# omnirevolve/omnirevolve-image-processor

Hardware: AMD Instinct MI355X
Metric: Mpx/s end-to-end (color->order) (higher is better)
Workload: dtype u8/i32 raster + f32/f64 geometry; 1 GPU; 4096x4096 BGR image, 8 colour layers, stages 02->12 (k-means fit, masks, edges, contours, scale, sort, intra dedup, cross dedup, plot order), default A4 canvas 8400x11880; parallelism=one GPU, one pipeline per colour layer, ops_last_step_rank0=4261, exchange=none

## Files before the change

### omnirevolve-image-processor_amd/csrc/orip_ctx.h

```cpp
#pragma once

#include <hip/hip_runtime.h>
#include <cstdint>
#include <cstdio>
#include <cstring>
#include <string>
#include <vector>
#include <map>
#include <mutex>
#include <atomic>
#include "../../include/orip.h"

typedef uint8_t u8;

#define ORIP_FAIL_AS(ctx, who, ...)                                      \
    do {                                                                 \
        char _b[512];                                                    \
        snprintf(_b, sizeof(_b), __VA_ARGS__);                           \
        { std::lock_guard<std::mutex> _g((ctx)->mu); (ctx)->err = std::string(who) + ": " + _b; } \
        return -1;                                                       \
    } while (0)
#define ORIP_FAIL(ctx, ...) ORIP_FAIL_AS(ctx, __func__, __VA_ARGS__)

#define HIPC_AS(ctx, who, call)                                                                \
// ... 72 lines not shown
    struct { void* pp; size_t off; } slot[CAP]; int n = 0; size_t total = 0;
    template <class T> void take(T*& ptr, size_t count, size_t align = 16) {
        if (alignof(T) > align) align = alignof(T);
        total = (total + align - 1) / align * align;
        if (n < CAP) { slot[n].pp = &ptr; slot[n].off = total; }
        n++; total += count * sizeof(T);
    }
    template <class... T> void each(size_t count, T*&... ptrs) { (take(ptrs, count), ...); }
    hipError_t commit(DBuf& buf, size_t tail_bytes) {
        const hipError_t e = n > CAP ? hipErrorInvalidValue : buf.ensure(total + tail_bytes);
        for (int i = 0; e == hipSuccess && i < n; i++) { void* a = (char*)buf.p + slot[i].off; memcpy(slot[i].pp, &a, sizeof a); }
        return e;
    }
};

struct LaneFlags {
    int not_binary;
    uint8_t palette[ORIP_MAX_LAYERS * 3];
    alignas(8) unsigned long long palette_counts[ORIP_MAX_LAYERS];
    alignas(8) unsigned long long label_counts[ORIP_MAX_LAYERS];
    int thin_changed[2];
    unsigned chain_counts[2];
    int trace_overflow;
    int nn_seed[2];
    alignas(8) unsigned long long nn_dbg2[10];
    int caps_overflow;
    unsigned caps_distinct;
    unsigned accept_survivors;
    alignas(8) unsigned long long accept_work;
    int zs_changed[12];
    unsigned comp_counts[3];
    int taps_kept;
    int plot_ops;
};
static_assert(sizeof(LaneFlags) <= 4096, "LaneRes::flags is 4096 bytes, allocated and zeroed by orip_create");

enum { VT0_KEYS = 0, VT0_HEADS = 1, VT0_COMP_START = 2, VT0_ORDER = 3, VT0_ORDER_SORT = 5, VT0_MEMO = 6, VT0_LOG_USED = 7, VT0_WINFO = 8, VT0_EDGE_BITS = 10,
       VT0_NMS_BITS = 11 };
enum { VTL_RANKS = 0,
       VTL_CUM = 1,
       VTL_SPLIT = 2,
       VTL_SAMPLES = 3,
       VTL_CAPS = 4,
       VTL_CELLS = 5,
       VTL_FEAT = 6,
       VTL_RUN_STARTS = 7,
       VTL_TAIL_RUNS = 8,
       VTL_STEPLOG = 9,
       VTL_SPLIT_FEAT = 10,
       VT_LEAVES = 11,
       VT_SLOTS = 12 };
struct LaneRes {
    hipStream_t stream = 0;
    hipStream_t stream2 = 0;
    hipEvent_t ev2 = nullptr, ev3 = nullptr, ev4 = nullptr;
    DBuf vtmp[VT_SLOTS], tmpE, tmpF, flags, canvas;
    DBuf pixbits;
    unsigned caps_hint = 0;
    hipEvent_t ev0 = nullptr, ev1 = nullptr;
    DPolys tp[6];
    struct Prefetch08 {
        bool pending = false;
        bool valid = false; uint64_t tag = 0; int64_t n = 0; int64_t tot_f = 0; double step = 0;
        const int64_t* src_off = nullptr;
        DBuf seg;
        DBuf feat, info, cum, ord;
// ... 130 lines not shown
```

### omnirevolve-image-processor_amd/csrc/vector08a.hip

```cpp
#include "vec08.h"
#include <rocprim/rocprim.hpp>
#include <type_traits>
#include <vector>

namespace {

template <class Src>
__global__ __launch_bounds__(128) void k_split_small08(Src src, int64_t n_polys, orip_params08 P, const PolyFeat* __restrict__ feat,
                                                        unsigned* __restrict__ is_tap, unsigned* __restrict__ is_keep, int2* __restrict__ tap_xy, GatherDesc* __restrict__ kd) {
    int64_t i = (int64_t)blockIdx.x * blockDim.x + threadIdx.x;
    if (i > n_polys) return;
    if (i == n_polys) { is_tap[i] = 0; is_keep[i] = 0; return; }
    const int64_t n = src.len(i);
    unsigned tap = 0, keep = 0;
    GatherDesc g; g.begin = src.off[i]; g.len = n; g.rev = 0; g.src = (int32_t)i;
    if (n >= 2) {
        const int32_t x0 = feat[i].x0, x1 = feat[i].x1, y0 = feat[i].y0, y1 = feat[i].y1;
        double d = (double)max(x1 - x0, y1 - y0);
        if (d <= P.tap_diam && d <= P.tap_max_dim && n <= (int64_t)P.tap_max_v) {
            double per; float cx, cy, r;
            if constexpr (std::is_same<Src, ESrc>::value) {
                const int32_t* p = reinterpret_cast<const int32_t*>(src.pts + src.off[i]);
                per = (double)vs::pairwise_seglen_sum<0>(p, n);
                if (per <= P.tap_max_per) vs::min_enclosing_circle(p, n, cx, cy, r);
            } else {
                auto cu = src.cur(i);
                LocalPts<decltype(cu), 64> lp; lp.load(cu, (int)n);
                per = (double)vs::pairwise_seglen_sum<0>(lp.xy, n);
                if (per <= P.tap_max_per) vs::min_enclosing_circle(lp.xy, n, cx, cy, r);
            }
            if (per <= P.tap_max_per) { tap = 1; tap_xy[i] = make_int2((int)vs::round_half_even((double)cx), (int)vs::round_half_even((double)cy)); }
        }
        if (!tap && !(d < P.min_keep)) {
// ... 368 lines not shown
    __syncthreads();
    const unsigned l0 = threadIdx.x * S;
    double v[S]; unsigned f[S];
#pragma unroll
    for (int q = 0; q < S; q++) { v[q] = shx[smp_slot8(l0 + q)]; f[q] = (b0 + l0 + q < MS) ? shr[smp_slot4(l0 + q)] >> 31 : 0u; }
    double wa = v[0]; unsigned wf = f[0];
#pragma unroll
    for (int q = 1; q < S; q++) { wa = f[q] ? v[q] : __dadd_rn(wa, v[q]); wf |= f[q]; }
    wave_seg_step<0x111, 0xf>(wa, wf); wave_seg_step<0x112, 0xf>(wa, wf); wave_seg_step<0x114, 0xf>(wa, wf); wave_seg_step<0x118, 0xf>(wa, wf);
    wave_seg_step<0x142, 0xa>(wa, wf); wave_seg_step<0x143, 0xc>(wa, wf);
    const int lane = threadIdx.x & 63, wv = threadIdx.x >> 6;
    if (lane == 63) { swa[wv] = wa; swf[wv] = wf; }
    double ea = __hiloint2double(__builtin_amdgcn_update_dpp(0, __double2hiint(wa), 0x138 , 0xf, 0xf, false),
                                 __builtin_amdgcn_update_dpp(0, __double2loint(wa), 0x138, 0xf, 0xf, false));
    const unsigned ef = (unsigned)__builtin_amdgcn_update_dpp(0, (int)wf, 0x138, 0xf, 0xf, false);
    __syncthreads();
    if (!ef) {
        double ca = 0.0;
        for (int k = 0; k < wv; k++) ca = swf[k] ? swa[k] : __dadd_rn(ca, swa[k]);
        ea = __dadd_rn(ca, ea);
    }
#pragma unroll
    for (int q = 0; q < S; q++) { ea = f[q] ? v[q] : __dadd_rn(ea, v[q]); v[q] = ea; }
    const unsigned gs = b0 + l0;
    if (gs + S <= MS) { double2* o = reinterpret_cast<double2*>(A.Sloc + gs); o[0] = make_double2(v[0], v[1]); o[1] = make_double2(v[2], v[3]); }
    else { for (int q = 0; q < S; q++) if (gs + q < MS) A.Sloc[gs + q] = v[q]; }
}

__device__ __forceinline__ double dpp_shr1_f64(double v) {
    const int lo = __builtin_amdgcn_update_dpp(0, __double2loint(v), 0x138 , 0xf, 0xf, true);
    const int hi = __builtin_amdgcn_update_dpp(0, __double2hiint(v), 0x138, 0xf, 0xf, true);
    return __hiloint2double(hi, lo);
}
__global__ __launch_bounds__(64) void k_tail_replay(const unsigned* __restrict__ sbase, int64_t n_rank, double T, SampleArrs A, unsigned* __restrict__ npop, const unsigned* __restrict__ only) {
    constexpr unsigned C = 1024u, RM = 2u * C - 1u;
    __shared__ double ops[64], rr[64];
    __shared__ double Dl[2 * C];
    __shared__ unsigned NPl[C];
    const int lane = threadIdx.x;
    for (int64_t r = blockIdx.x; r < n_rank; r += gridDim.x) {
        if (only && !only[r]) continue;
        const unsigned b = sbase[r], e = sbase[r + 1];
        if (e <= b) continue;
        const double* D = A.dprev + b; unsigned* NP = npop + b;
        const unsigned m = e - b;
        unsigned head = 0; double racc = 0.0;
        unsigned j0 = 0, cb = 0;
        auto fill = [&](unsigned c0) {
            double td[16]; unsigned tn[16];
#pragma unroll
            for (int u = 0; u < 16; u++) { const unsigned idx = c0 + (unsigned)lane + 64u * u; td[u] = D[idx < m ? idx : m - 1u]; tn[u] = NP[idx < m ? idx : m - 1u]; }
#pragma unroll
            for (int u = 0; u < 16; u++) { const unsigned idx = c0 + (unsigned)lane + 64u * u; Dl[idx & RM] = td[u]; NPl[idx & (C - 1u)] = tn[u]; }
        };
        auto dist = [&](unsigned idx) -> double { return (idx + C >= cb && idx < cb + C) ? Dl[idx & RM] : D[idx]; };
        auto plain = [&](unsigned s) {
            if (s > head) racc = __dadd_rn(racc, dist(s));
            while (head <= s && racc > T) { head++; if (head <= s) racc = __dsub_rn(racc, dist(head)); else racc = 0.0; }
            if (lane == 0) NP[s] = head;
        };
        fill(0);
        __syncthreads();
        while (j0 < m) {
            if (j0 >= cb + C) { __syncthreads(); cb += C; fill(cb); __syncthreads(); }
            const unsigned s = j0 + (unsigned)lane; const bool valid = s < m && s < cb + C;
            unsigned hp = valid ? NPl[s & (C - 1u)] : 0u;
            hp = hp > head ? hp : head;
            hp = wave_incl_scan_max_u32(hp);
            unsigned prevh = (unsigned)__builtin_amdgcn_update_dpp(0, (int)hp, 0x138 , 0xf, 0xf, true); if (lane == 0) prevh = head;
            const unsigned np = hp - prevh;
            const unsigned inc = valid ? 1u + np : 0u;
            unsigned off = wave_incl_scan_u32(inc);
            const unsigned long long fitm = __ballot(valid && off <= 64u);
            const int m_fit = __popcll(fitm);
            if (m_fit == 0) { plain(j0); j0++; continue; }
            const unsigned total = (unsigned)__builtin_amdgcn_readlane((int)off, m_fit - 1);
            off -= inc;
            if (lane < m_fit) {
                ops[off] = s > prevh ? dist(s) : 0.0;
                for (unsigned t = 0; t < np; t++) ops[off + 1u + t] = -dist(prevh + 1u + t);
            }
            __syncthreads();
            const double v = (unsigned)lane < total ? ops[lane] : 0.0;
            double d = lane == 0 ? __dadd_rn(racc, v) : v;
            double pre = d;
#pragma unroll
            for (int q = 1; q < 64; q++) pre = __dadd_rn(dpp_shr1_f64(pre), d);
            rr[lane] = pre;
            __syncthreads();
            bool bad = false;
            if (lane < m_fit) {
                const double after = rr[off + np];
                bad = after > T || (np > 0u && !(rr[off + np - 1u] > T)) || hp > s;
            }
            const unsigned long long badm = __ballot(bad);
            const int ncommit = badm ? __ffsll((long long)badm) - 1 : m_fit;
            if (lane < ncommit) NP[s] = hp;
            if (ncommit > 0) {
                head = (unsigned)__builtin_amdgcn_readlane((int)hp, ncommit - 1);
                const unsigned last_op = (unsigned)__builtin_amdgcn_readlane((int)(off + np), ncommit - 1);
                racc = rr[last_op];
            }
            __syncthreads();
            j0 += (unsigned)ncommit;
            if (badm) { plain(j0); j0++; }
        }
        __syncthreads();
    }
}

#define ORIP_TAIL_EPS 1e-6
#define ORIP_TAIL_BLOCKS 32u
__global__ __launch_bounds__(256) void k_tail_par(const unsigned* __restrict__ sbase, const unsigned* __restrict__ rank, const double* __restrict__ Sloc, unsigned MS, double T,
                                                   unsigned* __restrict__ npop, unsigned* __restrict__ redo) {
    __shared__ double win[512];
    const unsigned g0 = blockIdx.x * 256, w0 = g0 >= 256 ? g0 - 256 : 0;
    const unsigned KB = g0 / ORIP_SMP_BLOCK, B0 = KB * ORIP_SMP_BLOCK;
    const double lastprev = w0 < B0 ? Sloc[B0 - 1] : 0.0;
    for (unsigned t = threadIdx.x; t < 512; t += 256) {
        const unsigned idx = w0 + t;
        win[t] = (idx < MS && idx < g0 + 256) ? (idx < B0 ? Sloc[idx] - lastprev : Sloc[idx]) : 0.0;
    }
    __syncthreads();
    unsigned g = g0 + threadIdx.x;
    if (g >= MS) return;
    const unsigned r = rank[g], b = sbase[r];
    const double Sj = Sloc[g];
    bool unsure = !(Sj + (b < B0 ? lastprev : 0.0) < 4194304.0) || (g - b) >= (1u << 20);
    unsigned kc = KB; double acc = 0.0;
    auto tail = [&](unsigned p) -> double {
        if (p >= w0) return Sj - win[p - w0];
        const unsigned kb = p / ORIP_SMP_BLOCK;
        if (KB - kb > ORIP_TAIL_BLOCKS) { unsure = true; return __longlong_as_double(0x7ff0000000000000LL); }
        if (kb > kc) { kc = KB; acc = 0.0; }
        while (kc > kb) { kc--; acc += Sloc[kc * ORIP_SMP_BLOCK + (ORIP_SMP_BLOCK - 1u)]; }
        const double up = Sj + acc;
        if (!(up < 4194304.0)) unsure = true;
        return up - Sloc[p];
    };
    unsigned lo = b, hi = g;
    const unsigned wlo = max(b, w0);
    if (wlo == b || !(tail(wlo) <= T)) {
        if (wlo > b) lo = wlo + 1;
        else if (tail(b) <= T) hi = b;
        while (lo < hi) { const unsigned mid = (lo + hi) >> 1; if (tail(mid) <= T) hi = mid; else lo = mid + 1; }
    } else {
        hi = wlo;
        for (unsigned stepb = 1; hi > b; stepb <<= 1) {
            const unsigned p = (hi - b > stepb) ? hi - stepb : b;
            if (tail(p) <= T) { hi = p; if (p == b) break; } else { lo = p + 1; break; }
        }
        while (lo < hi) { const unsigned mid = (lo + hi) >> 1; if (tail(mid) <= T) hi = mid; else lo = mid + 1; }
    }
    const unsigned h = lo;
    if (!(tail(h) <= T - ORIP_TAIL_EPS)) unsure = true;
    if (h > b && !(tail(h - 1) > T + ORIP_TAIL_EPS)) unsure = true;
    npop[g] = h - b;
    if (unsure) redo[r] = 1u;
}
struct IncIndex {
    const unsigned* pxy;
    __device__ unsigned operator()(unsigned g) const { return pxy[g] != ORIP_PXY_OUT ? g + 1u : 0u; }
};
__global__ __launch_bounds__(256) void k_capprev(const unsigned* __restrict__ sbase, unsigned MS, SampleArrs A, const unsigned* __restrict__ lastin, int* __restrict__ capprev) {
    unsigned g = blockIdx.x * 256 + threadIdx.x;
    if (g >= MS) return;
    if (A.pxy[g] == ORIP_PXY_OUT) { capprev[g] = -2; return; }
    const unsigned b = sbase[A.rank[g]];
    const unsigned l = g > b ? lastin[g - 1] : 0u;
    capprev[g] = l ? (int)(l - 1u - b) : -1;
}

__device__ __forceinline__ unsigned long long cap_key(int x0, int y0, int x1, int y1) {
    unsigned long long a = ((unsigned long long)(unsigned)x0 << 14) | (unsigned)y0, b = ((unsigned long long)(unsigned)x1 << 14) | (unsigned)y1;
    if (b < a) { unsigned long long t = a; a = b; b = t; }
    return ((a << 28) | b) + 1ULL;
}
__device__ __forceinline__ unsigned long long hash64(unsigned long long x) { x ^= x >> 33; x *= 0xff51afd7ed558ccdULL; x ^= x >> 33; x *= 0xc4ceb9fe1a85ec53ULL; x ^= x >> 33; return x; }
struct __attribute__((aligned(16))) CapSlot { unsigned long long key; unsigned val; unsigned pad; };
__global__ __launch_bounds__(256) void k_caps_init(CapSlot* __restrict__ tab, unsigned long long tsize, LaneFlags* __restrict__ fl) {
    unsigned long long i = (unsigned long long)blockIdx.x * 256 + threadIdx.x;
    if (i == 0) { fl->caps_overflow = 0; fl->caps_distinct = 0u; fl->accept_survivors = 0u; fl->accept_work = 0ull; }
    if (i < tsize) reinterpret_cast<uint4*>(tab)[i] = make_uint4(0u, 0u, 0xffffffffu, 0u);
}
constexpr int ORIP_CAPSSET_PROBES = 4;
constexpr int ORIP_CAPSSET_SHIFT = 52;
template <bool CP>
__global__ __launch_bounds__(256) void k_caps_insert(SampleArrs A, const unsigned* __restrict__ sbase, const int* __restrict__ capprev, unsigned MS,
                                                      unsigned chunks, unsigned smask,
                                                      CapSlot* tab, unsigned long long tmask, int max_probe, int* __restrict__ overflow) {
    constexpr int S = 4;
// ... 364 lines not shown
        hipLaunchKernelGGL(k_pf_pick_info, dim3(cdiv(nk, 256)), dim3(256), 0, LN(c).stream, kept0.vview.as<VView>(), nk, F.info.as<RsInfo>(), F.n, F.src_off, F.src_off, F.tot_f, a.info, a.cumoff);
    } else {
        HIPC(c, hipMemcpyAsync(a.cumoff, kept0.off.p, (size_t)(nk + 1) * 8, hipMemcpyDeviceToDevice, LN(c).stream));
        { ProfScope ps(c, "k_cumlen"); ORIP_WITH_SRC(c, kept0, sv, { hipLaunchKernelGGL(k_cumlen<decltype(sv)>, dim3(cdiv(nk, 128)), dim3(128), 0, LN(c).stream, sv, nk, a.step, a.cum, a.info); }); }
        if (kept0.total > ORIP_LONG_CUM) { ProfScope ps(c, "k_cumlen_long"); ORIP_WITH_SRC(c, kept0, sv, {
                hipLaunchKernelGGL(k_cumlen_long2<decltype(sv)>, dim3((unsigned)std::min<int64_t>(nk, 8192), 1), dim3(64), 0, LN(c).stream, sv, nk, a.step, a.cum, (int64_t)0, a.info, a.ord, 0, (const float*)nullptr); }); }
    }
    T.tick("cumlen");
    hipLaunchKernelGGL(k_rank_counts, dim3(cdiv(nk + 1, 256)), dim3(256), 0, LN(c).stream, a.info, a.ord, nk, a.mr, a.feat, W, H, a.sbase + nk + 1, a.redo);
    ORIP_TRY(vscan_excl<unsigned>(c, a.mr, a.sbase, (size_t)nk + 1));
    unsigned ms_out[2] = {0, 0};
    ORIP_TRY(vread(c, ms_out, a.sbase + nk, 2));
    const unsigned MS = a.MS = ms_out[0]; a.any_out = ms_out[1] != 0 || getenv("ORIP_CAPPREV_SCAN");
    if (MS == 0) return 0;
    if (MS > 0x7ffffff0u) ORIP_FAIL(c, "too many samples");
    if (T.on) { char b[48]; snprintf(b, sizeof b, " [MS %u]", MS); T.log += b; }
    { Carve L; L.each(MS, a.A.sx, a.A.sy, a.A.dprev, a.A.pxy, a.A.rank, a.npop, a.capprev, a.sflag); HIPC(c, L.commit(LN(c).vtmp[VTL_SAMPLES], 1024)); }
    { Carve L; L.take(a.A.Sloc, MS); HIPC(c, L.commit(LN(c).vtmp[VTL_TAIL_RUNS], 64)); }
    const unsigned nb = (unsigned)cdiv(MS, 256);
    { Carve L; L.each(MS, a.ckin, a.ckout, a.cvin, a.cvout); L.take(a.hints, nb + 1, 64);
      HIPC(c, L.commit(LN(c).vtmp[VTL_CELLS], 64 + (size_t)MS * 8)); }
    a.cell = P.grid_stride > 0 ? P.grid_stride : std::max(4.0, P.col_rad); a.inv = 1.0 / a.cell;
    a.Wq = (W + 63) >> 6;
    HIPC(c, LN(c).canvas.ensure((size_t)W * H * 4 + 64));
    a.firstseq = LN(c).canvas.as<unsigned>();
    HIPC(c, LN(c).pixbits.ensure((size_t)a.Wq * H * 8 + 64));
    a.pixbits = LN(c).pixbits.as<unsigned long long>();
    HIPC(c, hipMemsetAsync(a.pixbits, 0, (size_t)a.Wq * H * 8, LN(c).stream));
    hipLaunchKernelGGL(k_sample_hints, dim3(cdiv(nb, 256)), dim3(256), 0, LN(c).stream, a.cumoff, a.cum, a.info, a.ord, a.sbase, nk, MS, a.step, nb, a.hints);
    { ProfScope ps(c, "k_samples"); ORIP_WITH_SRC(c, kept0, sv, { hipLaunchKernelGGL(k_samples<decltype(sv)>, dim3(cdiv(nb, 4)), dim3(256), 0, LN(c).stream, sv, a.cumoff, a.cum, a.info, a.ord, a.sbase, nk, MS, a.step, W, H, a.A, a.hints, (unsigned)nb, a.pixbits, a.Wq, a.firstseq); }); }
    T.tick("samples");
    return 0;
}
static void tail_dbg_dump(orip_ctx* c, int layer, const A08& a) {
    const int64_t nk = a.nk;
    std::vector<unsigned> h(nk), sb(nk + 1);
    hipStreamSynchronize(LN(c).stream);
    hipMemcpy(h.data(), a.redo, nk * 4, hipMemcpyDeviceToHost);
    hipMemcpy(sb.data(), a.sbase, (nk + 1) * 4, hipMemcpyDeviceToHost);
    unsigned long long nf = 0, sf = 0, mx = 0;
    for (int64_t q = 0; q < nk; q++) if (h[q]) { nf++; sf += sb[q + 1] - sb[q]; mx = std::max<unsigned long long>(mx, sb[q + 1] - sb[q]); }
    fprintf(stderr, "[tail dbg] layer %d: %llu of %lld polylines redone, %llu of %u samples, longest redone %llu\n", layer, nf, (long long)nk, sf, a.MS, mx);
}
static int a3_tails(orip_ctx* c, int layer, const orip_params08& P, A08& a) {
    const int64_t nk = a.nk; const unsigned MS = a.MS;
    {
        ProfScope ps(c, "k_tail_sim");
        hipLaunchKernelGGL(k_tail_par, dim3(cdiv(MS, 256)), dim3(256), 0, LN(c).stream, a.sbase, a.A.rank, a.A.Sloc, MS, P.tail_len_px, a.npop, a.redo);
        if (getenv("ORIP_TAIL_DBG")) tail_dbg_dump(c, layer, a);
        const unsigned* only = getenv("ORIP_TAIL_SEQ") ? nullptr : a.redo;
        HIPC(c, hipEventRecord(LN(c).ev2, LN(c).stream));
        HIPC(c, hipStreamWaitEvent(LN(c).stream2, LN(c).ev2, 0));
        hipLaunchKernelGGL(k_tail_replay, dim3((unsigned)std::min<int64_t>(nk, 65535)), dim3(64), 0, LN(c).stream2, a.sbase, nk, P.tail_len_px, a.A, a.npop, only);
        HIPC(c, hipEventRecord(LN(c).ev3, LN(c).stream2));
    }
    if (a.any_out) {
        unsigned* lastin = LN(c).vtmp[VTL_TAIL_RUNS].as<unsigned>();
        auto vin = rocprim::make_transform_iterator(rocprim::counting_iterator<unsigned>(0u), IncIndex{a.A.pxy});
        HIPC(c, orip_with_tmp(c, [&](void* tmp, size_t& bytes) { return rocprim::inclusive_scan_by_key(tmp, bytes, a.A.rank, vin, lastin, (size_t)MS, rocprim::maximum<unsigned>(), rocprim::equal_to<unsigned>(), LN(c).stream); }));
        hipLaunchKernelGGL(k_capprev, dim3(cdiv(MS, 256)), dim3(256), 0, LN(c).stream, a.sbase, MS, a.A, lastin, a.capprev);
    }
    else a.capprev = nullptr;
    return 0;
}
static int a4_capsules(orip_ctx* c, const orip_params08& P, A08& a) {
    const unsigned MS = a.MS; LaneFlags* fl = LN(c).flags.as<LaneFlags>();
    unsigned long long tfull = 1024; while (tfull < 2ull * MS) tfull <<= 1;
    unsigned long long tsize = 1024;
    if (LN(c).caps_hint) { while (tsize < 3ull * LN(c).caps_hint) tsize <<= 1; } else { while (tsize < MS / 4ull) tsize <<= 1; }
    tsize = std::min(tsize, tfull);
    if (getenv("ORIP_CAPS_TINY")) tsize = 1024;
    static const unsigned cand[] = {8192u, 4096u, 2048u, 1024u};
    unsigned R = 1024u, TS = 2048u;
    for (unsigned r : cand) if (cdiv(MS, r) >= 2048 || r == 1024u) { R = r; break; }
    if (const char* e = getenv("ORIP_CAPS_RANGE")) {
        char* end = nullptr; const unsigned long r = strtoul(e, &end, 10); unsigned long t = TS;
        if (end && *end == ':') t = strtoul(end + 1, nullptr, 10);
        if (r < 1024 || r > 65536 || (r & 1023)) ORIP_FAIL(c, "ORIP_CAPS_RANGE: a multiple of 1024 up to 65536");
        if (t < 32 || t > 4096 || (t & (t - 1))) ORIP_FAIL(c, "ORIP_CAPS_RANGE: a power of two from 32 to 4096 slots");
        R = (unsigned)r; TS = (unsigned)t;
    }
    if (getenv("ORIP_CAPSSET_TINY")) TS = 32u;
    const unsigned lds = TS * 12u;
    CapSlot* tab = nullptr;
    int* d_ovf = &fl->caps_overflow; unsigned* d_dist = &fl->caps_distinct;
    for (;; tsize = std::min(tfull, tsize * 4)) {
        HIPC(c, LN(c).vtmp[VTL_CAPS].ensure((size_t)tsize * 16 + 64));
// ... 67 lines not shown
```

### omnirevolve-image-processor_amd/csrc/vector08b.hip

```cpp
#include "vec08.h"
#include "bitplane.h"
#include <cstdio>
#define PAD8 64

namespace {

__global__ __launch_bounds__(256) void k_iota(int* a, int n) { int i = blockIdx.x * 256 + threadIdx.x; if (i < n) a[i] = i; }
__global__ __launch_bounds__(256) void k_bbox_pairs(const PolyFeat* __restrict__ f, int n, int exp, int* __restrict__ par) {
    for (int i = blockIdx.x; i < n; i += gridDim.x) {
        int ax0 = f[i].x0 - exp, ay0 = f[i].y0 - exp, ax1 = f[i].x1 + exp, ay1 = f[i].y1 + exp;
        for (int j = i + 1 + threadIdx.x; j < n; j += 256) {
            int bx0 = f[j].x0 - exp, by0 = f[j].y0 - exp, bx1 = f[j].x1 + exp, by1 = f[j].y1 + exp;
            if (!(ax1 < bx0 || bx1 < ax0 || ay1 < by0 || by1 < ay0)) uf_unite(par, i, j);
        }
    }
}
struct GroupInfo { int x0, y0, x1, y1; unsigned long long longest; unsigned long long near0, near1; int rank; int a0x, a0y, a1x, a1y; };
__global__ __launch_bounds__(256) void k_group_init(GroupInfo* g, int n) {
    int i = blockIdx.x * 256 + threadIdx.x; if (i >= n) return;
    GroupInfo q; q.x0 = q.y0 = 0x7fffffff; q.x1 = q.y1 = -0x7fffffff; q.longest = ~0ULL; q.near0 = q.near1 = ~0ULL; q.rank = -1; q.a0x = q.a0y = q.a1x = q.a1y = 0;
    g[i] = q;
}
__global__ __launch_bounds__(256) void k_group_accum(const PolyFeat* __restrict__ f, int n, int exp, int* __restrict__ par, GroupInfo* __restrict__ g, unsigned* __restrict__ is_root) {
    int i = blockIdx.x * 256 + threadIdx.x; if (i > n) return;
// ... 48 lines not shown
    if (any) any_s = 1;
    __syncthreads();
    const bool empty = !any_s;
    int cur = 0;
    if (!empty) {
        for (int t = 0; t < 2 * iters; t++) {
            int del_core = 0;
            for (int i = tid; i < ZS_ROWS * 4; i += 256) {
                const int r = i >> 2, wx = i & 3;
                const unsigned long long M = T[cur][r][wx];
                unsigned long long out = 0;
                if (M) {
                    auto G = [&](int rr, int ww) -> unsigned long long { return (rr < 0 || rr >= ZS_ROWS || ww < 0 || ww > 3) ? 0ULL : T[cur][rr][ww]; };
                    const unsigned long long del = zs_delete<ZS_STANDARD>(M, nb8_of(M, G(r - 1, wx), G(r - 1, wx - 1), G(r - 1, wx + 1), G(r, wx - 1), G(r, wx + 1), G(r + 1, wx), G(r + 1, wx - 1), G(r + 1, wx + 1)), t & 1);
                    out = M & ~del;
                    if (del && r >= ZS_HALO && r < ZS_HALO + ZS_TR && (wx == 1 || wx == 2)) del_core = 1;
                }
                T[cur ^ 1][r][wx] = out;
            }
            if (del_core) changed[t >> 1] = 1;
            cur ^= 1;
            __syncthreads();
        }
    }
    for (int i = tid; i < ZS_TR * 2; i += 256) {
        const int r = ZS_HALO + (i >> 1), wx = 1 + (i & 1), y = y0 + r, xw = x0 + wx;
        if (y < H && xw < Ww) d[(size_t)y * Ww + xw] = empty ? 0ULL : T[cur][r][wx];
    }
}
__device__ __forceinline__ unsigned long long wave_min_u64(unsigned long long v) {
    for (int o = 32; o > 0; o >>= 1) { unsigned long long t = __shfl_xor(v, o, 64); if (t < v) v = t; }
    return v;
}
__global__ __launch_bounds__(256) void k_nearest_anchor(const unsigned* __restrict__ lin, int64_t m, const unsigned* __restrict__ gid, int Wp, GroupInfo* __restrict__ g) {
    int64_t i = (int64_t)blockIdx.x * 256 + threadIdx.x;
    const bool valid = i < m;
    unsigned grp = 0; unsigned long long k0 = ~0ULL, k1 = ~0ULL;
    if (valid) {
        unsigned p = lin[i]; int x = (int)(p % Wp) - PAD8, y = (int)(p / Wp) - PAD8;
        grp = gid[p] - 1;
        const GroupInfo* G = g + grp;
        long long d0 = (long long)(y - G->a0y) * (y - G->a0y) + (long long)(x - G->a0x) * (x - G->a0x);
        long long d1 = (long long)(y - G->a1y) * (y - G->a1y) + (long long)(x - G->a1x) * (x - G->a1x);
        k0 = ((unsigned long long)d0 << 27) | p; k1 = ((unsigned long long)d1 << 27) | p;
    }
    unsigned long long rem = __ballot(valid);
    const int lane = threadIdx.x & 63;
    while (rem) {
        int L = __ffsll((long long)rem) - 1;
        unsigned gL = (unsigned)__shfl((int)grp, L, 64);
        bool same = valid && grp == gL;
        unsigned long long m0 = wave_min_u64(same ? k0 : ~0ULL), m1 = wave_min_u64(same ? k1 : ~0ULL);
        if (lane == L) {
            GroupInfo* G = g + gL;
            if (m0 < *(volatile unsigned long long*)&G->near0) atomicMin(&G->near0, m0);
            if (m1 < *(volatile unsigned long long*)&G->near1) atomicMin(&G->near1, m1);
        }
        rem &= ~__ballot(same);
    }
}
__global__ __launch_bounds__(128) void k_comp_keys(const unsigned* __restrict__ cs, unsigned nc, const unsigned* __restrict__ lin, const unsigned* __restrict__ gid, int Wp,
                                                    const GroupInfo* __restrict__ g, unsigned long long* __restrict__ ckey, unsigned* __restrict__ cidx) {
    unsigned c = blockIdx.x * blockDim.x + threadIdx.x; if (c >= nc) return;
    unsigned b = cs[c], e = cs[c + 1];
    const GroupInfo* G = g + (gid[lin[b]] - 1);
    int w = max(1, G->x1 - G->x0); int wb = (w + 1) >> 1;
    unsigned best = 0xffffffffu;
    for (unsigned q = b; q < e; q++) {
        unsigned p = lin[q]; int x = (int)(p % Wp) - PAD8 - G->x0, y = (int)(p / Wp) - PAD8 - G->y0;
        unsigned k = (unsigned)((y >> 1) * wb + (x >> 1));
        best = min(best, k);
    }
    ckey[c] = ((unsigned long long)(unsigned)G->rank << 32) | best; cidx[c] = c;
}

__device__ const int OFY[8] = {-1, -1, -1, 0, 1, 1, 1, 0};
__device__ const int OFX[8] = {-1, 0, 1, 1, 1, 0, -1, -1};

__global__ __launch_bounds__(256) void k_cid_fill(const unsigned* __restrict__ lin, unsigned m, unsigned* __restrict__ cid) {
    unsigned q = blockIdx.x * 256 + threadIdx.x; if (q < m) cid[lin[q]] = q;
}
__global__ __launch_bounds__(256) void k_nbr_build(const unsigned* __restrict__ lin, unsigned m, const u8* __restrict__ sk, const unsigned* __restrict__ cid, int Wp, int Hp, unsigned* __restrict__ nbr) {
    size_t t = (size_t)blockIdx.x * 256 + threadIdx.x; if (t >= (size_t)m * 8) return;
    unsigned q = (unsigned)(t >> 3); int k = (int)(t & 7);
    unsigned p = lin[q]; int y = (int)(p / Wp) + OFY[k], x = (int)(p % Wp) + OFX[k];
    unsigned v = ~0u;
    if (y >= 0 && y < Hp && x >= 0 && x < Wp) { size_t j = (size_t)y * Wp + x; if (sk[j]) v = cid[j]; }
    nbr[t] = v;
}
__global__ __launch_bounds__(256) void k_comp_classes(const unsigned* __restrict__ corder, unsigned nc, const unsigned* __restrict__ cs, unsigned cap0, unsigned cap1, int need,
                                                      unsigned* __restrict__ counts, unsigned* __restrict__ l0, unsigned* __restrict__ l1, unsigned* __restrict__ l2, unsigned* __restrict__ outcnt) {
    unsigned oi = blockIdx.x * 256 + threadIdx.x; if (oi >= nc) return;
    unsigned c = corder[oi]; unsigned s = cs[c + 1] - cs[c];
    outcnt[oi] = 0;
    if ((int)s < need) return;
    if (s <= cap0) l0[atomicAdd(&counts[0], 1u)] = oi;
    else if (s <= cap1) l1[atomicAdd(&counts[1], 1u)] = oi;
    else l2[atomicAdd(&counts[2], 1u)] = oi;
}

template <bool LDSV> struct CompWork;
template <> struct CompWork<true> {
    typedef uint16_t Id; typedef ushort2 Stk;
    static constexpr unsigned NONE = 0xffffu;
    Id* nb; Id* prev; Id* que; float* cum; u8* seen; float2* P; Stk* stk; u8* keep;
    __device__ __forceinline__ unsigned nbr_of(unsigned u, int k) const { return nb[u * 8 + k]; }
// ... 261 lines not shown
    return 0;
}
static int b_components(orip_ctx* c, B08& b, PhaseTimer& T) {
    const int Wp = b.Wp, Hp = b.Hp, Wwp = b.Wwp; const size_t nwords = b.nwords;
    dim3 blk(256); const dim3 gwd((unsigned)cdiv((int64_t)nwords, 256));
    HIPC(c, LN(c).vtmp[VTL_SPLIT_FEAT].ensure(b.Np * 4 + 64));
    int* L2 = LN(c).vtmp[VTL_SPLIT_FEAT].as<int>();
    hipLaunchKernelGGL(k_ccl_bits<IdsLinear>, gwd, blk, 0, LN(c).stream, b.bA, L2, Hp, Wp, Wwp, 0);
    { ProfScope ps(c, "k_ccl2_merge"); hipLaunchKernelGGL(k_ccl_bits<IdsLinear>, gwd, blk, 0, LN(c).stream, b.bA, L2, Hp, Wp, Wwp, 1); }
    hipLaunchKernelGGL(k_ccl_bits<IdsLinear>, gwd, blk, 0, LN(c).stream, b.bA, L2, Hp, Wp, Wwp, 2);
    T.tick("c:ccl");
    const int nblk = (int)cdiv((int64_t)nwords, 256);
    unsigned *bc, *bo; { Carve L; L.each(nblk + 1, bc, bo); HIPC(c, L.commit(LN(c).vtmp[VTL_RANKS], 64)); }
    HIPC(c, hipMemsetAsync(bc + nblk, 0, 4, LN(c).stream));
    bp_compact_count(LN(c).stream, (unsigned)nblk, b.bA, nwords, bc);
    ORIP_TRY(vscan_excl<unsigned>(c, bc, bo, (size_t)nblk + 1));
    b.M = 0; ORIP_TRY(vread(c, &b.M, bo + nblk));
    const unsigned M = b.M;
    if (M == 0) return 0;
    unsigned *kin, *lin_in;
    { Carve L; L.each(M, kin, lin_in, b.keys, b.lin); HIPC(c, L.commit(LN(c).vtmp[VTL_CUM], 64)); }
    hipLaunchKernelGGL(k_compact_write_bits<Emit08>, dim3(nblk), blk, 0, LN(c).stream, b.bA, nwords, bo, Emit08{L2, Wp, Wwp}, kin, lin_in);
    ORIP_TRY((vsort_pairs<unsigned, unsigned>(c, kin, b.keys, lin_in, b.lin, (size_t)M, 0, 27)));
    unsigned *head, *hs; { Carve L; L.each((size_t)M + 1, head, hs); HIPC(c, L.commit(LN(c).vtmp[VTL_SAMPLES], 64)); }
    bp_heads(LN(c).stream, b.keys, (int64_t)M, (int64_t)M + 1, head);
    ORIP_TRY(vscan_excl<unsigned>(c, head, hs, (size_t)M + 1));
    b.NC = 0; ORIP_TRY(vread(c, &b.NC, hs + M));
    const unsigned NC = b.NC; const size_t nc1 = (size_t)NC + 1;
    unsigned long long *ckin, *ckout; unsigned* cidx;
    { Carve L; L.each(nc1, ckin, ckout); L.take(b.cs, nc1 + 1);
      L.each(nc1, cidx, b.corder, b.outcnt, b.oflag, b.oscan); L.take(b.pd, NC); HIPC(c, L.commit(LN(c).vtmp[VTL_CAPS], 256)); }
    bp_comp_starts(LN(c).stream, head, hs, (int64_t)M, b.cs, NC);
    T.tick("c:sort");
    hipLaunchKernelGGL(k_nearest_anchor, dim3(cdiv(M, 256)), blk, 0, LN(c).stream, b.lin, (int64_t)M, b.gid, Wp, b.grp);
    T.tick("c:anchor");
    hipLaunchKernelGGL(k_comp_keys, dim3(cdiv(NC, 128)), dim3(128), 0, LN(c).stream, b.cs, NC, b.lin, b.gid, Wp, b.grp, ckin, cidx);
    ORIP_TRY((vsort_pairs<unsigned long long, unsigned>(c, ckin, ckout, cidx, b.corder, (size_t)NC, 0, 64)));
    T.tick("comps");
    return 0;
}
static int b_paths(orip_ctx* c, const orip_params08& P, B08& b, DPolys& merged, PhaseTimer& T) {
    const int Wp = b.Wp, Hp = b.Hp; const size_t Np = b.Np; const unsigned M = b.M, NC = b.NC; const size_t nc1 = (size_t)NC + 1;
    dim3 blk(256);
    const double stp = P.post_step;
    const double ratio = 1.41422 / stp;
    const unsigned omul = ratio > 1.0 ? 2u : 1u;
    const double pass = std::min(stp, 65536.0);
    auto pcap_of = [&](unsigned cap) { return (unsigned)(cap * ratio) + std::min((unsigned)pass, cap) + 4u; };
    auto cap_of = [&](size_t budget) {
        const double a = ((double)budget - 13.0 * (pass + 4.0) - 64.0) / (25.0 + 13.0 * ratio), b2 = ((double)budget - 13.0 * 4.0 - 64.0) / (25.0 + 13.0 * (ratio + 1.0));
        const double cap = std::max(a, b2);
        return (unsigned)std::min(cap, 65000.0) & ~7u;
    };
    const size_t lds0 = 32 * 1024, lds1 = 160 * 1024;
    unsigned cap0 = cap_of(lds0), cap1 = cap_of(lds1);
    if (const char* ov = getenv("ORIP_COMP_CAPS")) {
        unsigned a = 0, b2 = 0; if (sscanf(ov, "%u,%u", &a, &b2) == 2 && a >= 8 && a <= b2) { cap0 = std::min(cap0, a & ~7u); cap1 = std::min(cap1, b2 & ~7u); }
    }
    auto lds_bytes = [&](unsigned cap) { return (size_t)cap * 25 + (size_t)pcap_of(cap) * 13 + 16; };
    unsigned *cid, *nbr, *l0, *l1, *l2; int2* outpts; CompScratch X;
    { Carve L; L.take(cid, Np); L.take(nbr, (size_t)M * 8); L.each(M, X.prev, X.que, X.cum); L.each((size_t)M * omul, X.P, X.stk);
      L.take(outpts, (size_t)M * omul); L.each(nc1, l0, l1, l2); L.take(X.seen, M); L.take(X.keep, (size_t)M * omul); HIPC(c, L.commit(LN(c).vtmp[VTL_CELLS], 1024)); }
    unsigned* counts = LN(c).flags.as<LaneFlags>()->comp_counts;
    HIPC(c, hipMemsetAsync(counts, 0, sizeof(LaneFlags::comp_counts), LN(c).stream));
    hipLaunchKernelGGL(k_cid_fill, dim3(cdiv(M, 256)), blk, 0, LN(c).stream, b.lin, M, cid);
    hipLaunchKernelGGL(k_nbr_build, dim3((unsigned)cdiv((int64_t)M * 8, 256)), blk, 0, LN(c).stream, b.lin, M, b.skA, cid, Wp, Hp, nbr);
    hipLaunchKernelGGL(k_comp_classes, dim3(cdiv(NC, 256)), blk, 0, LN(c).stream, b.corder, NC, b.cs, cap0, cap1, std::max(2, P.post_minlen), counts, l0, l1, l2, b.outcnt);
    CompArgs A; A.corder = b.corder; A.cs = b.cs; A.lin = b.lin; A.gid = b.gid; A.g = b.grp; A.cid = cid; A.nbr = nbr; A.Wp = Wp; A.min_len = P.post_minlen; A.step = stp;
    A.eps = (float)P.post_eps; A.omul = omul; A.outpts = outpts; A.outcnt = b.outcnt;
// ... 43 lines not shown
```

Baseline: 287.0 Mpx/s.

## Use exact integer scan in tail replay, stop early, parallelize component keys

The tail replay kernel now tries an exact fixed-point integer prefix scan across the wave, built on DPP compose steps, in place of the 63-step serial f64 DPP add chain. It falls back to the old chain when the integer window does not hold. k_tail_par records the last unsure sample index so replay can stop there instead of replaying the whole polyline. Component key computation moves from one thread per component looping over its pixels to one thread per pixel with a segmented wave min and atomicMin, and k_nearest_anchor initializes the keys. Debug counters and dumps are added behind environment variables, and the code must preserve bit-exact rounding semantics.

Measured after the change: 293.3 Mpx/s (median of 6 runs). 2.2% higher.

```diff
diff --git a/omnirevolve-image-processor_amd/csrc/orip_ctx.h b/omnirevolve-image-processor_amd/csrc/orip_ctx.h
--- a/omnirevolve-image-processor_amd/csrc/orip_ctx.h
+++ b/omnirevolve-image-processor_amd/csrc/orip_ctx.h
@@ -128,6 +128,7 @@
     unsigned comp_counts[3];
     int taps_kept;
     int plot_ops;
+    alignas(8) unsigned long long tail_dbg[4];
 };
 static_assert(sizeof(LaneFlags) <= 4096, "LaneRes::flags is 4096 bytes, allocated and zeroed by orip_create");
 
diff --git a/omnirevolve-image-processor_amd/csrc/tail_window.h b/omnirevolve-image-processor_amd/csrc/tail_window.h
--- /dev/null
+++ b/omnirevolve-image-processor_amd/csrc/tail_window.h
@@ -0,0 +1,57 @@
+#pragma once
+#include <math.h>
+#include <stdint.h>
+#if defined(__HIPCC__)
+#define TW_FN __host__ __device__ __forceinline__
+#else
+#define TW_FN inline
+#endif
+
+struct TwInc { long long ev, od; };
+
+TW_FN unsigned long long tw_bits(double x) { unsigned long long b; __builtin_memcpy(&b, &x, 8); return b; }
+TW_FN double tw_double(unsigned long long b) { double x; __builtin_memcpy(&x, &b, 8); return x; }
+TW_FN bool tw_frame(double p, int& e, long long& P) {
+    const unsigned long long b = tw_bits(p), ef = b >> 52;
+    if (ef < 123u || ef > 1923u) return false;
+    e = (int)ef - 1023; P = (long long)((b & 0xfffffffffffffull) | (1ull << 52));
+    return true;
+}
+TW_FN bool tw_inc(double d, int e, TwInc& f) {
+    f.ev = f.od = 0;
+    if (d == 0.0) return true;
+    const unsigned long long ef = (tw_bits(d) >> 52) & 0x7ffu;
+    if (ef == 0u || ef == 0x7ffu) return false;
+    const double s = d * tw_double((unsigned long long)(52 - e + 1023) << 52);
+    if (!(fabs(s) < 9007199254740992.0)) return false;
+    const double r = rint(s);
+    if (fabs(s - r) == 0.5) {
+        const long long m = (long long)floor(s), odd = m & 1;
+        f.ev = m + odd; f.od = m + 1 - odd;
+    } else f.ev = f.od = (long long)r;
+    return true;
+}
+TW_FN TwInc tw_compose(TwInc f, TwInc g) {
+    TwInc h;
+    h.ev = f.ev + ((f.ev & 1) ? g.od : g.ev);
+    h.od = f.od + ((f.od & 1) ? g.ev : g.od);
+    return h;
+}
+TW_FN long long tw_apply(long long P, TwInc f) { return P + ((P & 1) ? f.od : f.ev); }
+TW_FN bool tw_inside(long long S) { return S > (1ll << 52) && S < (1ll << 53); }
+TW_FN double tw_value(long long S, int e) { return tw_double(((unsigned long long)(e + 1023) << 52) | ((unsigned long long)S & 0xfffffffffffffull)); }
+
+inline int tw_window(double p, const double* ops, int n, double* out) {
+    int e; long long P;
+    if (!tw_frame(p, e, P)) return 0;
+    TwInc acc = {0, 0};
+    for (int i = 0; i < n; i++) {
+        TwInc f;
+        if (!tw_inc(ops[i], e, f)) return i;
+        acc = tw_compose(acc, f);
+        const long long S = tw_apply(P, acc);
+        if (!tw_inside(S)) return i;
+        out[i] = tw_value(S, e);
+    }
+    return n;
+}
diff --git a/omnirevolve-image-processor_amd/csrc/vector08a.hip b/omnirevolve-image-processor_amd/csrc/vector08a.hip
--- a/omnirevolve-image-processor_amd/csrc/vector08a.hip
+++ b/omnirevolve-image-processor_amd/csrc/vector08a.hip
@@ -1,4 +1,5 @@
 #include "vec08.h"
+#include "tail_window.h"
 #include <rocprim/rocprim.hpp>
 #include <type_traits>
 #include <vector>
@@ -433,20 +434,37 @@
     const int hi = __builtin_amdgcn_update_dpp(0, __double2hiint(v), 0x138, 0xf, 0xf, true);
     return __hiloint2double(hi, lo);
 }
-__global__ __launch_bounds__(64) void k_tail_replay(const unsigned* __restrict__ sbase, int64_t n_rank, double T, SampleArrs A, unsigned* __restrict__ npop, const unsigned* __restrict__ only) {
+template <int CTRL, int ROWMASK>
+__device__ __forceinline__ void wave_tw_step(TwInc& f) {
+    auto sh = [](long long x) -> long long {
+        const int lo = __builtin_amdgcn_update_dpp(0, (int)(unsigned)((unsigned long long)x & 0xffffffffull), CTRL, ROWMASK, 0xf, false);
+        const int hi = __builtin_amdgcn_update_dpp(0, (int)(unsigned)((unsigned long long)x >> 32), CTRL, ROWMASK, 0xf, false);
+        return (long long)(((unsigned long long)(unsigned)hi << 32) | (unsigned)lo);
+    };
+    TwInc p; p.ev = sh(f.ev); p.od = sh(f.od);
+    f = tw_compose(p, f);
+}
+__device__ __forceinline__ void wave_incl_scan_tw(TwInc& f) {
+    wave_tw_step<0x111, 0xf>(f); wave_tw_step<0x112, 0xf>(f); wave_tw_step<0x114, 0xf>(f); wave_tw_step<0x118, 0xf>(f);
+    wave_tw_step<0x142, 0xa>(f); wave_tw_step<0x143, 0xc>(f);
+}
+__global__ __launch_bounds__(64) void k_tail_replay(const unsigned* __restrict__ sbase, int64_t n_rank, double T, SampleArrs A, unsigned* __restrict__ npop, const unsigned* __restrict__ only,
+                                                    unsigned long long* __restrict__ dbg) {
     constexpr unsigned C = 1024u, RM = 2u * C - 1u;
     __shared__ double ops[64], rr[64];
     __shared__ double Dl[2 * C];
     __shared__ unsigned NPl[C];
     const int lane = threadIdx.x;
     for (int64_t r = blockIdx.x; r < n_rank; r += gridDim.x) {
-        if (only && !only[r]) continue;
+        const unsigned stop = only ? only[r] : 0xffffffffu;
+        if (!stop) continue;
         const unsigned b = sbase[r], e = sbase[r + 1];
         if (e <= b) continue;
         const double* D = A.dprev + b; unsigned* NP = npop + b;
-        const unsigned m = e - b;
+        const unsigned m = e - b, me = min(m, stop);
         unsigned head = 0; double racc = 0.0;
         unsigned j0 = 0, cb = 0;
+        unsigned n_rounds = 0, n_round_smp = 0, n_plain = 0, n_exact = 0;
         auto fill = [&](unsigned c0) {
             double td[16]; unsigned tn[16];
 #pragma unroll
@@ -459,12 +477,13 @@
             if (s > head) racc = __dadd_rn(racc, dist(s));
             while (head <= s && racc > T) { head++; if (head <= s) racc = __dsub_rn(racc, dist(head)); else racc = 0.0; }
             if (lane == 0) NP[s] = head;
+            n_plain++;
         };
         fill(0);
         __syncthreads();
-        while (j0 < m) {
+        while (j0 < me) {
             if (j0 >= cb + C) { __syncthreads(); cb += C; fill(cb); __syncthreads(); }
-            const unsigned s = j0 + (unsigned)lane; const bool valid = s < m && s < cb + C;
+            const unsigned s = j0 + (unsigned)lane; const bool valid = s < me && s < cb + C;
             unsigned hp = valid ? NPl[s & (C - 1u)] : 0u;
             hp = hp > head ? hp : head;
             hp = wave_incl_scan_max_u32(hp);
@@ -483,10 +502,21 @@
             }
             __syncthreads();
             const double v = (unsigned)lane < total ? ops[lane] : 0.0;
-            double d = lane == 0 ? __dadd_rn(racc, v) : v;
-            double pre = d;
-#pragma unroll
-            for (int q = 1; q < 64; q++) pre = __dadd_rn(dpp_shr1_f64(pre), d);
+            double pre; bool exact = false;
+            { int fe; long long fP;
+              if (tw_frame(racc, fe, fP)) {
+                  TwInc f; const bool fine = tw_inc(v, fe, f);
+                  wave_incl_scan_tw(f);
+                  const long long S = tw_apply(fP, f);
+                  exact = !__ballot((unsigned)lane < total && !(fine && tw_inside(S)));
+                  pre = tw_value(S, fe);
+              } }
+            if (!exact) {
+                const double d = lane == 0 ? __dadd_rn(racc, v) : v;
+                pre = d;
+#pragma unroll
+                for (int q = 1; q < 64; q++) pre = __dadd_rn(dpp_shr1_f64(pre), d);
+            } else n_exact++;
             rr[lane] = pre;
             __syncthreads();
             bool bad = false;
@@ -503,9 +533,10 @@
                 racc = rr[last_op];
             }
             __syncthreads();
-            j0 += (unsigned)ncommit;
+            j0 += (unsigned)ncommit; n_rounds++; n_round_smp += (unsigned)ncommit;
             if (badm) { plain(j0); j0++; }
         }
+        if (dbg && lane == 0) { atomicAdd(&dbg[0], (unsigned long long)n_rounds); atomicAdd(&dbg[1], (unsigned long long)n_round_smp); atomicAdd(&dbg[2], (unsigned long long)n_plain); atomicAdd(&dbg[3], (unsigned long long)n_exact); }
         __syncthreads();
     }
 }
@@ -513,7 +544,7 @@
 #define ORIP_TAIL_EPS 1e-6
 #define ORIP_TAIL_BLOCKS 32u
 __global__ __launch_bounds__(256) void k_tail_par(const unsigned* __restrict__ sbase, const unsigned* __restrict__ rank, const double* __restrict__ Sloc, unsigned MS, double T,
-                                                   unsigned* __restrict__ npop, unsigned* __restrict__ redo) {
+                                                   unsigned* __restrict__ npop, unsigned* __restrict__ redo, unsigned* __restrict__ dbg_first) {
     __shared__ double win[512];
     const unsigned g0 = blockIdx.x * 256, w0 = g0 >= 256 ? g0 - 256 : 0;
     const unsigned KB = g0 / ORIP_SMP_BLOCK, B0 = KB * ORIP_SMP_BLOCK;
@@ -557,7 +588,10 @@
     if (!(tail(h) <= T - ORIP_TAIL_EPS)) unsure = true;
     if (h > b && !(tail(h - 1) > T + ORIP_TAIL_EPS)) unsure = true;
     npop[g] = h - b;
-    if (unsure) redo[r] = 1u;
+    if (unsure) {
+        atomicMax(&redo[r], 1u + (g - b));
+        if (dbg_first) atomicMin(&dbg_first[r], g - b);
+    }
 }
 struct IncIndex {
     const unsigned* pxy;
@@ -988,27 +1022,47 @@
     T.tick("samples");
     return 0;
 }
-static void tail_dbg_dump(orip_ctx* c, int layer, const A08& a) {
+static void tail_dbg_dump(orip_ctx* c, int layer, const A08& a, const unsigned* first) {
     const int64_t nk = a.nk;
-    std::vector<unsigned> h(nk), sb(nk + 1);
+    std::vector<unsigned> h(nk), sb(nk + 1), f(nk);
     hipStreamSynchronize(LN(c).stream);
     hipMemcpy(h.data(), a.redo, nk * 4, hipMemcpyDeviceToHost);
     hipMemcpy(sb.data(), a.sbase, (nk + 1) * 4, hipMemcpyDeviceToHost);
-    unsigned long long nf = 0, sf = 0, mx = 0;
-    for (int64_t q = 0; q < nk; q++) if (h[q]) { nf++; sf += sb[q + 1] - sb[q]; mx = std::max<unsigned long long>(mx, sb[q + 1] - sb[q]); }
-    fprintf(stderr, "[tail dbg] layer %d: %llu of %lld polylines redone, %llu of %u samples, longest redone %llu\n", layer, nf, (long long)nk, sf, a.MS, mx);
+    hipMemcpy(f.data(), first, nk * 4, hipMemcpyDeviceToHost);
+    unsigned long long nf = 0, sf = 0, mx = 0, upto = 0;
+    std::vector<int64_t> red;
+    for (int64_t q = 0; q < nk; q++) if (h[q]) { nf++; sf += sb[q + 1] - sb[q]; upto += h[q]; mx = std::max<unsigned long long>(mx, sb[q + 1] - sb[q]); red.push_back(q); }
+    fprintf(stderr, "[tail dbg] layer %d: %llu of %lld polylines redone, %llu of %u samples (%llu up to the last unsure one), longest redone %llu\n", layer, nf, (long long)nk, sf, a.MS, upto, mx);
+    std::stable_sort(red.begin(), red.end(), [&](int64_t x, int64_t y) { return sb[x + 1] - sb[x] > sb[y + 1] - sb[y]; });
+    for (size_t i = 0; i < red.size() && i < 5; i++) { const int64_t q = red[i];
+        fprintf(stderr, "[tail dbg]   rank %lld: %u samples, first unsure %u, last unsure %u\n", (long long)q, sb[q + 1] - sb[q], f[q], h[q] - 1u); }
+}
+static void tail_dbg_replay(orip_ctx* c, int layer, const unsigned long long* dbg) {
+    unsigned long long v[4] = {0, 0, 0, 0};
+    hipStreamSynchronize(LN(c).stream2);
+    hipMemcpy(v, dbg, sizeof v, hipMemcpyDeviceToHost);
+    fprintf(stderr, "[tail dbg] layer %d: replay %llu rounds, %llu samples committed by rounds, %llu by the plain loop, %llu rounds in the integer form\n", layer, v[0], v[1], v[2], v[3]);
 }
 static int a3_tails(orip_ctx* c, int layer, const orip_params08& P, A08& a) {
     const int64_t nk = a.nk; const unsigned MS = a.MS;
     {
         ProfScope ps(c, "k_tail_sim");
-        hipLaunchKernelGGL(k_tail_par, dim3(cdiv(MS, 256)), dim3(256), 0, LN(c).stream, a.sbase, a.A.rank, a.A.Sloc, MS, P.tail_len_px, a.npop, a.redo);
-        if (getenv("ORIP_TAIL_DBG")) tail_dbg_dump(c, layer, a);
+        const bool dbg = getenv("ORIP_TAIL_DBG") != nullptr;
+        unsigned* dbg_first = nullptr; unsigned long long* dbg_cnt = nullptr;
+        if (dbg) {
+            HIPC(c, hipMalloc(&dbg_first, (size_t)(nk + 1) * 4));
+            const hipError_t me = hipMemsetAsync(dbg_first, 0xff, (size_t)(nk + 1) * 4, LN(c).stream);
+            if (me != hipSuccess) { hipFree(dbg_first); HIPC(c, me); }
+            dbg_cnt = LN(c).flags.as<LaneFlags>()->tail_dbg;
+        }
+        hipLaunchKernelGGL(k_tail_par, dim3(cdiv(MS, 256)), dim3(256), 0, LN(c).stream, a.sbase, a.A.rank, a.A.Sloc, MS, P.tail_len_px, a.npop, a.redo, dbg_first);
+        if (dbg) { tail_dbg_dump(c, layer, a, dbg_first); hipFree(dbg_first); HIPC(c, hipMemsetAsync(dbg_cnt, 0, sizeof(LaneFlags::tail_dbg), LN(c).stream)); }
         const unsigned* only = getenv("ORIP_TAIL_SEQ") ? nullptr : a.redo;
         HIPC(c, hipEventRecord(LN(c).ev2, LN(c).stream));
         HIPC(c, hipStreamWaitEvent(LN(c).stream2, LN(c).ev2, 0));
-        hipLaunchKernelGGL(k_tail_replay, dim3((unsigned)std::min<int64_t>(nk, 65535)), dim3(64), 0, LN(c).stream2, a.sbase, nk, P.tail_len_px, a.A, a.npop, only);
+        hipLaunchKernelGGL(k_tail_replay, dim3((unsigned)std::min<int64_t>(nk, 65535)), dim3(64), 0, LN(c).stream2, a.sbase, nk, P.tail_len_px, a.A, a.npop, only, dbg_cnt);
         HIPC(c, hipEventRecord(LN(c).ev3, LN(c).stream2));
+        if (dbg) tail_dbg_replay(c, layer, dbg_cnt);
     }
     if (a.any_out) {
         unsigned* lastin = LN(c).vtmp[VTL_TAIL_RUNS].as<unsigned>();
diff --git a/omnirevolve-image-processor_amd/csrc/vector08b.hip b/omnirevolve-image-processor_amd/csrc/vector08b.hip
--- a/omnirevolve-image-processor_amd/csrc/vector08b.hip
+++ b/omnirevolve-image-processor_amd/csrc/vector08b.hip
@@ -104,9 +104,11 @@
     for (int o = 32; o > 0; o >>= 1) { unsigned long long t = __shfl_xor(v, o, 64); if (t < v) v = t; }
     return v;
 }
-__global__ __launch_bounds__(256) void k_nearest_anchor(const unsigned* __restrict__ lin, int64_t m, const unsigned* __restrict__ gid, int Wp, GroupInfo* __restrict__ g) {
+__global__ __launch_bounds__(256) void k_nearest_anchor(const unsigned* __restrict__ lin, int64_t m, const unsigned* __restrict__ gid, int Wp, GroupInfo* __restrict__ g,
+                                                        unsigned long long* __restrict__ ckey, unsigned nc) {
     int64_t i = (int64_t)blockIdx.x * 256 + threadIdx.x;
     const bool valid = i < m;
+    if (i < nc) ckey[i] = ~0ULL;
     unsigned grp = 0; unsigned long long k0 = ~0ULL, k1 = ~0ULL;
     if (valid) {
         unsigned p = lin[i]; int x = (int)(p % Wp) - PAD8, y = (int)(p / Wp) - PAD8;
@@ -131,19 +133,31 @@
         rem &= ~__ballot(same);
     }
 }
-__global__ __launch_bounds__(128) void k_comp_keys(const unsigned* __restrict__ cs, unsigned nc, const unsigned* __restrict__ lin, const unsigned* __restrict__ gid, int Wp,
+__global__ __launch_bounds__(256) void k_comp_keys(const unsigned* __restrict__ cs, const unsigned* __restrict__ head, const unsigned* __restrict__ head_scan, unsigned m,
+                                                    const unsigned* __restrict__ lin, const unsigned* __restrict__ gid, int Wp,
                                                     const GroupInfo* __restrict__ g, unsigned long long* __restrict__ ckey, unsigned* __restrict__ cidx) {
-    unsigned c = blockIdx.x * blockDim.x + threadIdx.x; if (c >= nc) return;
-    unsigned b = cs[c], e = cs[c + 1];
-    const GroupInfo* G = g + (gid[lin[b]] - 1);
-    int w = max(1, G->x1 - G->x0); int wb = (w + 1) >> 1;
-    unsigned best = 0xffffffffu;
-    for (unsigned q = b; q < e; q++) {
+    const unsigned q = blockIdx.x * 256 + threadIdx.x;
+    const bool valid = q < m;
+    unsigned c = 0xffffffffu; unsigned long long key = ~0ULL;
+    if (valid) {
+        const unsigned hd = head[q];
+        c = head_scan[q] + hd - 1u;
+        const GroupInfo* G = g + (gid[lin[cs[c]]] - 1);
+        int w = max(1, G->x1 - G->x0); int wb = (w + 1) >> 1;
         unsigned p = lin[q]; int x = (int)(p % Wp) - PAD8 - G->x0, y = (int)(p / Wp) - PAD8 - G->y0;
         unsigned k = (unsigned)((y >> 1) * wb + (x >> 1));
-        best = min(best, k);
-    }
-    ckey[c] = ((unsigned long long)(unsigned)G->rank << 32) | best; cidx[c] = c;
+        key = ((unsigned long long)(unsigned)G->rank << 32) | k;
+        if (hd) cidx[c] = c;
+    }
+    const int lane = threadIdx.x & 63;
+    for (int o = 1; o < 64; o <<= 1) {
+        const unsigned long long t = __shfl_up(key, o, 64); const unsigned ct = (unsigned)__shfl_up((int)c, o, 64);
+        if (lane >= o && ct == c && t < key) key = t;
+    }
+    const unsigned cn = (unsigned)__shfl_down((int)c, 1, 64);
+    if (valid && (lane == 63 || cn != c)) {
+        if (key < *(volatile unsigned long long*)&ckey[c]) atomicMin(&ckey[c], key);
+    }
 }
 
 __device__ const int OFY[8] = {-1, -1, -1, 0, 1, 1, 1, 0};
@@ -471,9 +485,15 @@
       L.each(nc1, cidx, b.corder, b.outcnt, b.oflag, b.oscan); L.take(b.pd, NC); HIPC(c, L.commit(LN(c).vtmp[VTL_CAPS], 256)); }
     bp_comp_starts(LN(c).stream, head, hs, (int64_t)M, b.cs, NC);
     T.tick("c:sort");
-    hipLaunchKernelGGL(k_nearest_anchor, dim3(cdiv(M, 256)), blk, 0, LN(c).stream, b.lin, (int64_t)M, b.gid, Wp, b.grp);
+    hipLaunchKernelGGL(k_nearest_anchor, dim3(cdiv(M, 256)), blk, 0, LN(c).stream, b.lin, (int64_t)M, b.gid, Wp, b.grp, ckin, NC);
     T.tick("c:anchor");
-    hipLaunchKernelGGL(k_comp_keys, dim3(cdiv(NC, 128)), dim3(128), 0, LN(c).stream, b.cs, NC, b.lin, b.gid, Wp, b.grp, ckin, cidx);
+    hipLaunchKernelGGL(k_comp_keys, dim3(cdiv(M, 256)), blk, 0, LN(c).stream, b.cs, head, hs, M, b.lin, b.gid, Wp, b.grp, ckin, cidx);
+    if (getenv("ORIP_COMP_DBG")) {
+        std::vector<unsigned long long> hk(NC);
+        hipStreamSynchronize(LN(c).stream);
+        hipMemcpy(hk.data(), ckin, (size_t)NC * 8, hipMemcpyDeviceToHost);
+        for (unsigned q = 0; q < NC; q++) fprintf(stderr, "[comp dbg] rank %u block %u\n", (unsigned)(hk[q] >> 32), (unsigned)hk[q]);
+    }
     ORIP_TRY((vsort_pairs<unsigned long long, unsigned>(c, ckin, ckout, cidx, b.corder, (size_t)NC, 0, 64)));
     T.tick("comps");
     return 0;
```
